# SewoongLab/PLeaS-Merging

Hardware: AMD Instinct MI355X
Metric: wall-clock (s): ResNet-101 pair, 100-batch act-match + 400-step PLeaS, 1/8 GPU (lower is better)
Workload: dtype f32

## Files before the change

include/pleas_hip.h:

```cpp
#ifndef PLEAS_HIP_H
#define PLEAS_HIP_H

#include <stddef.h>
#include <stdint.h>

#ifdef __cplusplus
extern "C" {
#endif

#define PLEAS_OK 0
#define PLEAS_EINVAL (-22)
#define PLEAS_ENOMEM (-12)
#define PLEAS_EHIP (-5)

const char* pleas_version(void);
const char* pleas_last_error(void);

#define PLEAS_EPI_INNER 0
#define PLEAS_EPI_NEG_CDIST 1
size_t pleas_gram_ws_bytes(int B, int C, int64_t HW);
int pleas_gram_accum(const float* x, const float* y, int B, int C, int64_t HW, int epilogue, int accumulate,
                     float* acc, void* ws, size_t ws_bytes, void* stream);

typedef struct pleas_gram_node {
// ... 10 lines not shown
    const float* scale_y;
    const float* shift_y;
} pleas_gram_node;
size_t pleas_gram_batch_ws_bytes(const pleas_gram_node* nodes, int n_nodes, const int* group_C, int n_groups);
int pleas_gram_batch(const pleas_gram_node* nodes, int n_nodes, float* const* group_acc, const int* group_C,
                     int n_groups, int epilogue, int accumulate, void* ws, size_t ws_bytes, int ws_fresh, void* stream);

#define PLEAS_LSAP_MAX_N 4096
int pleas_lsap_batched(const float* const* cost, const int* n, int nprob, int maximize, int64_t* const* col_ind,
                       void* stream);
int pleas_lsap_host(const void* cost, int is_double, int n, int maximize, int64_t* col_ind);

size_t pleas_bottleneck_ws_bytes(const int* n, int nprob);
int pleas_bottleneck_batched(const float* const* cost, const int* n, int nprob, int maximize, int64_t* const* col_ind,
                             float* t_out, void* ws, size_t ws_bytes, void* stream);
int pleas_bottleneck_host(const void* cost, int is_double, int n, int maximize, int64_t* col_ind, double* t_out);

int pleas_merge_blocks(const float* w1, const float* w2, float* out, int64_t outer, int rows_out, int cols_out,
                       int64_t inner, int rows_src, int cols_src, const int32_t* row1, const int32_t* row2,
                       const int32_t* col1, const int32_t* col2, int n_merged_rows, void* stream);

typedef struct pleas_merge_item {
    const float* w1;
    const float* w2;
    float* out;
    const int32_t* row1;
    const int32_t* row2;
    int64_t outer, inner;
    int rows_out, rows_src, n_merged;
    int sub_stride, sub_h, sub_w;
} pleas_merge_item;
size_t pleas_merge_batch_ws_bytes(const pleas_merge_item* items, int n_items);
int pleas_merge_batch(const pleas_merge_item* items, int n_items, void* ws, size_t ws_bytes, int ws_fresh, void* stream);

int pleas_bn_act(const float* x, const float* scale, const float* shift, const float* res, float* y, int64_t n,
                 int channels, int64_t inner, int relu, void* stream);
int pleas_bn_act_tracked(const float* x, const float* scale, const float* shift, const float* res, float* y_bn,
                         float* y_sum, float* y, int64_t n, int channels, int64_t inner, int relu, void* stream);

int pleas_bn_act_tracked_batches(const float* x, const float* scale, const float* shift, const float* res, float* y_bn,
                                 float* y_sum, float* y, int64_t n_per_batch, int batches, int channels, int64_t inner,
                                 int relu, void* stream);

int pleas_bn_act_maxpool(const float* x, const float* scale, const float* shift, float* y, int64_t n, int channels, int H,
                         int W, int KH, int KW, int stride, int pad, int relu, void* stream);

int pleas_pool_gather(const float* x, const int32_t* src, float* y, int64_t N, int C, int64_t HW, int K, void* stream);

int pleas_top1_count(const float* logits, const int64_t* labels, int64_t N, int C, int64_t* hits, int64_t* pred, void* stream);

int pleas_softmax_xent(const float* logits, const int64_t* labels, int64_t N, int C, float scale, float* dlogits,
                       float* row_loss, float* loss, int64_t* counts, void* stream);

size_t pleas_bn_train_ws_bytes(int64_t n, int channels);
int pleas_bn_train_fold(const float* x, int64_t n, int channels, int64_t inner, const float* gamma, const float* beta,
                        double eps, double momentum, float* running_mean, float* running_var,
                        int64_t* num_batches_tracked, float* scale, float* shift, void* ws, size_t ws_bytes,
                        void* stream);
int pleas_bn_train_fold_batches(const float* x, int64_t n, int batches, int channels, int64_t inner, const float* gamma,
                                const float* beta, double eps, double momentum, float* running_mean, float* running_var,
                                int64_t* num_batches_tracked, float* scale, float* shift, void* ws, size_t ws_bytes,
                                void* stream);

int pleas_masked_adam(float* p, const float* g, const float* mask, float* m, float* v, int64_t n, float lr,
                      float b1, float b2, float eps, int step, void* stream);

// ... 112 lines not shown
```

pleas_merging_amd/_lib.py:

```python
from __future__ import annotations

import ctypes
import os
from ctypes import POINTER, c_char_p, c_float, c_int, c_int64, c_size_t, c_void_p
from typing import Optional

_LIB: Optional[ctypes.CDLL] = None
LIB_PATH = os.path.join(os.path.dirname(os.path.abspath(__file__)), "csrc", "libpleas_hip.so")

EPI_INNER, EPI_NEG_CDIST = 0, 1
ARITH_FP32, ARITH_SPLIT_BF16, ARITH_SPLIT_BF16_EXACT = 0, 1, 2
LSAP_MAX_N = 4096
IMAGE_NHWC, IMAGE_NCHW = 0, 1

SIGNATURES = {
    "pleas_version": (c_char_p, []),
    "pleas_last_error": (c_char_p, []),
    "pleas_gram_ws_bytes": (c_size_t, [c_int, c_int, c_int64]),
    "pleas_gram_accum": (c_int, [c_void_p, c_void_p, c_int, c_int, c_int64, c_int, c_int, c_void_p, c_void_p, c_size_t,
                                 c_void_p]),
    "pleas_lsap_batched": (c_int, [POINTER(c_void_p), POINTER(c_int), c_int, c_int, POINTER(c_void_p), c_void_p]),
    "pleas_lsap_host": (c_int, [c_void_p, c_int, c_int, c_int, c_void_p]),
    "pleas_bottleneck_ws_bytes": (c_size_t, [POINTER(c_int), c_int]),
    "pleas_bottleneck_batched": (c_int, [POINTER(c_void_p), POINTER(c_int), c_int, c_int, POINTER(c_void_p), c_void_p, c_void_p,
                                         c_size_t, c_void_p]),
    "pleas_bottleneck_host": (c_int, [c_void_p, c_int, c_int, c_int, c_void_p, c_void_p]),
    "pleas_merge_blocks": (c_int, [c_void_p, c_void_p, c_void_p, c_int64, c_int, c_int, c_int64, c_int, c_int, c_void_p,
                                   c_void_p, c_void_p, c_void_p, c_int, c_void_p]),
    "pleas_merge_batch_ws_bytes": (c_size_t, [c_void_p, c_int]),
    "pleas_merge_batch": (c_int, [c_void_p, c_int, c_void_p, c_size_t, c_int, c_void_p]),
    "pleas_bn_act": (c_int, [c_void_p, c_void_p, c_void_p, c_void_p, c_void_p, c_int64, c_int, c_int64, c_int, c_void_p]),
    "pleas_bn_act_tracked": (c_int, [c_void_p, c_void_p, c_void_p, c_void_p, c_void_p, c_void_p, c_void_p, c_int64, c_int,
                                     c_int64, c_int, c_void_p]),
    "pleas_bn_act_maxpool": (c_int, [c_void_p, c_void_p, c_void_p, c_void_p, c_int64, c_int, c_int, c_int, c_int, c_int, c_int,
                                     c_int, c_int, c_void_p]),
    "pleas_bn_act_tracked_batches": (c_int, [c_void_p, c_void_p, c_void_p, c_void_p, c_void_p, c_void_p, c_void_p, c_int64, c_int,
                                             c_int, c_int64, c_int, c_void_p]),
    "pleas_bn_train_fold_batches": (c_int, [c_void_p, c_int64, c_int, c_int, c_int64, c_void_p, c_void_p, ctypes.c_double,
                                            ctypes.c_double, c_void_p, c_void_p, c_void_p, c_void_p, c_void_p, c_void_p,
                                            c_size_t, c_void_p]),
    "pleas_bn_train_ws_bytes": (c_size_t, [c_int64, c_int]),
    "pleas_bn_train_fold": (c_int, [c_void_p, c_int64, c_int, c_int64, c_void_p, c_void_p, ctypes.c_double, ctypes.c_double,
                                    c_void_p, c_void_p, c_void_p, c_void_p, c_void_p, c_void_p, c_size_t, c_void_p]),
    "pleas_masked_adam": (c_int, [c_void_p, c_void_p, c_void_p, c_void_p, c_void_p, c_int64, c_float, c_float, c_float,
                                  c_float, c_int, c_void_p]),
    "pleas_sqerr_ws_bytes": (c_size_t, [c_int64]),
    "pleas_sqerr": (c_int, [c_void_p, c_void_p, c_int64, c_float, c_int, c_void_p, c_float, c_void_p, c_void_p, c_size_t,
                            c_void_p]),
    "pleas_channel_sum": (c_int, [c_void_p, c_int, c_int, c_int64, c_void_p, c_void_p]),
    "pleas_linear_ws_bytes": (c_size_t, [c_int64, c_int, c_int]),
    "pleas_linear_plan_info": (c_int, [c_int64, c_int, c_int, POINTER(c_int)]),
    "pleas_linear_fwd": (c_int, [c_void_p, c_void_p, c_void_p, c_void_p, c_int64, c_int, c_int, c_void_p, c_size_t, c_void_p]),
    "pleas_column_sum": (c_int, [c_void_p, c_int64, c_int, c_void_p, c_void_p]),
    "pleas_image_batch": (c_int, [c_void_p, c_void_p, c_void_p, c_void_p, c_void_p, c_int64] + [c_int] * 6 + [c_void_p]),
    "pleas_resample_plan_bytes": (c_size_t, [c_void_p, c_int64, c_int, c_int]),
    "pleas_resample_plan": (c_int, [c_void_p, c_void_p, c_int64, c_int, c_int, c_int, c_int64, c_void_p, c_size_t]),
    "pleas_resample_plan_info": (c_int, [c_void_p, c_size_t, POINTER(c_int64)]),
    "pleas_image_resample_host": (c_int, [c_void_p, c_void_p, c_size_t, c_void_p, c_void_p, c_void_p, c_void_p]),
    "pleas_image_resample": (c_int, [c_void_p, c_void_p, c_void_p, c_size_t, c_void_p, c_void_p, c_void_p, c_void_p, c_size_t,
                                     c_void_p]),
    "pleas_prof_enable": (None, [c_int]),
    "pleas_prof_select": (None, [ctypes.c_uint]),
    "pleas_prof_reset": (None, []),
# ... 95 lines not shown
```

pleas_merging_amd/csrc/common.hpp:

```cpp
#pragma once
#include <hip/hip_runtime.h>

#include <cstdint>
#include <cstdio>
#include <algorithm>
#include <cstdlib>
#include <cstring>
#include <vector>

#include "pleas_hip.h"

namespace pleas {

extern thread_local char g_last_error[256];

inline int hip_fail(hipError_t e, const char* what) {
    std::snprintf(g_last_error, sizeof(g_last_error), "%s: %s", what, hipGetErrorString(e));
    return PLEAS_EHIP;
}

inline int bad_arg(const char* what) {
    std::snprintf(g_last_error, sizeof(g_last_error), "invalid argument: %s", what);
    return PLEAS_EINVAL;
}
// ... 144 lines not shown
            if (t.bytes) PLEAS_HIP_CHECK(hipMemcpyAsync((char*)ws + t.offset, t.host, t.bytes, hipMemcpyHostToDevice, stream));
        PLEAS_HIP_CHECK(hipStreamSynchronize(stream));
        p.uploaded = true;
        return PLEAS_OK;
    }
};

template <int N>
struct SideStreams {
    struct Set {
        hipStream_t streams[N];
        hipEvent_t forked, joined[N];
        bool ok = false;
    };
    static constexpr int kMaxDev = 16;
    Set sets[kMaxDev], none;
    bool tried[kMaxDev] = {false};
    Set& current() {
        int dev = 0;
        if (hipGetDevice(&dev) != hipSuccess || dev < 0 || dev >= kMaxDev) return none;
        Set& s = sets[dev];
        if (!tried[dev]) {
            tried[dev] = true;
            bool ok = hipEventCreateWithFlags(&s.forked, hipEventDisableTiming) == hipSuccess;
            for (int i = 0; ok && i < N; ++i)
                ok = hipStreamCreateWithFlags(&s.streams[i], hipStreamNonBlocking) == hipSuccess &&
                     hipEventCreateWithFlags(&s.joined[i], hipEventDisableTiming) == hipSuccess;
            s.ok = ok;
        }
        return s;
    }
};

template <class Item>
struct XcdWork {
    double w;
    int64_t key;
    Item it;
};
template <class Item>
inline std::vector<Item> xcd_order_items(std::vector<XcdWork<Item>>& work, const Item& noop, bool by_default = true) {
    std::vector<Item> out;
    const char* env = std::getenv("PLEAS_XCD_ORDER");
    if (env ? env[0] == '0' : !by_default) {
        std::stable_sort(work.begin(), work.end(), [](const XcdWork<Item>& a, const XcdWork<Item>& b) { return a.w > b.w; });
        for (auto& x : work) out.push_back(x.it);
        return out;
    }
    struct Group { double total = 0, longest = 0; std::vector<size_t> idx; };
    std::vector<Group> groups;
    {
        std::vector<size_t> order(work.size());
        for (size_t i = 0; i < work.size(); ++i) order[i] = i;
        std::stable_sort(order.begin(), order.end(), [&](size_t a, size_t b) { return work[a].key < work[b].key; });
        int64_t last = 0;
        for (size_t n = 0; n < order.size(); ++n) {
            const size_t i = order[n];
            if (n == 0 || work[i].key != last) groups.emplace_back();
            last = work[i].key;
            Group& g = groups.back();
            g.total += work[i].w;
            g.longest = std::max(g.longest, work[i].w);
            g.idx.push_back(i);
        }
    }
    std::stable_sort(groups.begin(), groups.end(), [](const Group& a, const Group& b) { return a.total > b.total; });
// ... 27 lines not shown
```

pleas_merging_amd/csrc/conv_fwd.hip:

```cpp
#include <algorithm>
#include <mutex>
#include <vector>

#include "fwd_schedule.hpp"
#include "nt_tile.hpp"

namespace pleas {

typedef short s16x4_t __attribute__((ext_vector_type(4)));
typedef short s16x8_t __attribute__((ext_vector_type(8)));

constexpr int fTN = 128;

enum class FwdMode : int { Fit = 0, Conv = 1, ConvImage = 2, Image = 3, ConvStats = 4 };
constexpr int fModes = 5;
constexpr bool fwd_has_target(FwdMode m) { return m == FwdMode::Fit; }
constexpr bool fwd_has_image(FwdMode m) { return m == FwdMode::ConvImage || m == FwdMode::Image; }
constexpr bool fwd_stores_y(FwdMode m) { return m != FwdMode::Image; }
constexpr bool fwd_has_stats(FwdMode m) { return m == FwdMode::ConvStats; }

struct FwdLayerDev {
    const float* ip;
    const float* w;
    const float* bias;
// ... 893 lines not shown
    d.KH = l.KH; d.KW = l.KW; d.stride = l.stride; d.pad = l.pad; d.Csrc = l.Csrc; d.n_merged = l.n_merged;
    d.HWo = (uint32_t)HWo; d.Ptot = (uint32_t)Ptot; d.Kd = (uint32_t)Kd;
    d.dscale = l.dscale;
    const int TM = l.Cout > 64 ? 128 : 64;
    d.variant = (TM == 64 ? 1 : 0) | (Kd % 4 == 0 ? 0 : 2);
    if (l.flags & PLEAS_FWD_KPOS_MAJOR) {
        if (l.Cin % kBK != 0) return bad_arg("conv_fwd: kernel-position-major weights need Cin % 32 == 0");
        d.variant |= 4;
    }
    lds_bytes = (size_t)(2 * TM * kLds + 2 * fTN * kLds) * sizeof(float);
    {
        const int R = l.KH * l.KW;
        const bool same = l.stride == 1 && l.KH == l.KW && (l.KH & 1) && l.pad == (l.KH - 1) / 2;
        const int halo = l.pad * (l.Win + 1);
        const int kind = R > 1 ? 2 : (HWo % 4 == 0 ? 0 : 1);
        const int Lr = kind == 2 ? fFlatColsK : fFlatRow1;
        const size_t flat_lds = std::max((size_t)(2 * TM * kLds + (kind == 2 ? fFlatColsK * fFlatPix : 2 * kBK * Lr)) * sizeof(float),
                                         (size_t)TM * 132 * sizeof(float));
        if (same && l.Cin % kBK == 0 && R <= 32 && (R == 1 || (l.flags & PLEAS_FWD_KPOS_MAJOR)) &&
            fTN + 2 * halo < Lr && flat_lds <= lds_bytes && (int64_t)l.N * l.Cin * HWo < (1ll << 32)) {
            d.variant |= 8 | (kind << 4);
            lds_bytes = flat_lds;
            if (arith_mode() != 0 && kind != 1) {
                const size_t img = (size_t)(TM * kSplitRow + (kind == 2 ? fFlatColsK * kSplitRow : 3 * kBK * fSplitPixRow)) * sizeof(__bf16);
                lds_bytes = std::max(img, (size_t)TM * 132 * sizeof(float));
            }
        }
    }
    TM_out = TM;
    return PLEAS_OK;
}

static std::mutex g_fplan_mu;

static int build_fwd_plan(FwdPlan& P, const pleas_fwd_layer* ly, int n) {
    P.split = arith_mode();
    P.layers.assign(n, FwdLayerDev());
    P.items.clear();
    for (int f = 0; f < fForms; ++f) P.form_begin[f] = P.form_count[f] = 0;
    P.loss.assign(n, FwdLossDev());
    P.flops = P.bytes = 0;
    std::vector<XcdWork<FwdItemDev>> work[fForms];
    double form_work[fForms] = {0};
    for (int f = 0; f < fForms; ++f) P.form_lds[f] = 0;
    int parts = 0;
    for (int i = 0; i < n; ++i) {
        const pleas_fwd_layer& l = ly[i];
        FwdLayerDev& d = P.layers[i];
        size_t lds_bytes = 0;
        int TM = 128;
        if (const int rc = fwd_describe(l, d, lds_bytes, TM); rc != PLEAS_OK) return rc;
        const int64_t Ptot = d.Ptot, Kd = d.Kd;
        d.part_base = parts;
        const int tms = (int)ceil_div(l.Cout, TM), tps = (int)ceil_div(Ptot, fTN);
        int slot = 0;
        const int form = fwd_form_of(d.variant);
        for (int tp = 0; tp < tps; ++tp)
            for (int tm = 0; tm < tms; ++tm) {
                XcdWork<FwdItemDev> w;
                w.it = FwdItemDev{i, tm, tp, slot++};
                w.w = (double)ceil_div(Kd, kBK) * TM;
                w.key = (int64_t)i * 65536 + tp / 32;
                work[form].push_back(w);
                form_work[form] += w.w;
            }
        P.loss[i] = FwdLossDev{parts, slot, l.loss_scale, 0};
// ... 301 lines not shown
```

pleas_merging_amd/csrc/merge_batch.hip:

```cpp
#include <algorithm>
#include <mutex>
#include <vector>

#include "common.hpp"

namespace pleas {

typedef float f32x4 __attribute__((ext_vector_type(4)));

constexpr int mThreads = 256;
constexpr int mUnroll = 4;
constexpr int mSpan = mThreads * mUnroll;

struct MergeItemDev {
    const float* w1;
    const float* w2;
    float* out;
    const int32_t* row1;
    const int32_t* row2;
    uint32_t total_v;
    uint32_t inner_v;
    uint32_t rows_out, rows_src;
    int n_merged, vec;
    int first_block;
    int stride;
    uint32_t w_out, w_src, inner_src, pad;
};

__global__ __launch_bounds__(mThreads) void merge_batch_kernel(const MergeItemDev* __restrict__ items,
                                                               const int* __restrict__ block_item) {
    const MergeItemDev it = items[block_item[blockIdx.x]];
    const uint32_t base = (uint32_t)(blockIdx.x - it.first_block) * mSpan + threadIdx.x;
    uint32_t idx[mUnroll];
    int r1[mUnroll], r2[mUnroll];
    uint32_t o_[mUnroll], iv_[mUnroll], r_[mUnroll];
#pragma unroll
    for (int u = 0; u < mUnroll; ++u) {
        idx[u] = base + u * mThreads;
        const uint32_t id = min(idx[u], it.total_v - 1);
        const uint32_t t = id / it.inner_v;
        iv_[u] = id - t * it.inner_v;
        o_[u] = t / it.rows_out;
        r_[u] = t - o_[u] * it.rows_out;
        r1[u] = PLEAS_GLOBAL_I(it.row1)[r_[u]];
        r2[u] = PLEAS_GLOBAL_I(it.row2)[r_[u]];
    }
    if (it.vec == 4) {
        f32x4 a[mUnroll], b[mUnroll];
#pragma unroll
        for (int u = 0; u < mUnroll; ++u) {
            const size_t oa = ((size_t)o_[u] * it.rows_src + max(r1[u], 0)) * it.inner_v + iv_[u];
            const size_t ob = ((size_t)o_[u] * it.rows_src + max(r2[u], 0)) * it.inner_v + iv_[u];
            a[u] = reinterpret_cast<const __attribute__((address_space(1))) f32x4*>(PLEAS_GLOBAL(it.w1))[oa];
            b[u] = reinterpret_cast<const __attribute__((address_space(1))) f32x4*>(PLEAS_GLOBAL(it.w2))[ob];
        }
#pragma unroll
        for (int u = 0; u < mUnroll; ++u) {
            if (idx[u] >= it.total_v) continue;
            const float coef = (int)r_[u] < it.n_merged ? 0.5f : 1.0f;
            f32x4 q;
#pragma unroll
            for (int e = 0; e < 4; ++e) q[e] = ((r1[u] >= 0 ? a[u][e] : 0.f) + (r2[u] >= 0 ? b[u][e] : 0.f)) * coef;
            reinterpret_cast<__attribute__((address_space(1))) f32x4*>(PLEAS_GLOBAL_W(it.out))[idx[u]] = q;
        }
    } else {
        float a[mUnroll], b[mUnroll];
#pragma unroll
        for (int u = 0; u < mUnroll; ++u) {
            uint32_t src = iv_[u], row_len = it.inner_v;
            if (it.stride > 0) {
                const uint32_t oh = iv_[u] / it.w_out, ow = iv_[u] - oh * it.w_out;
                src = (oh * it.w_src + ow) * (uint32_t)it.stride;
                row_len = it.inner_src;
            }
            a[u] = PLEAS_GLOBAL(it.w1)[((size_t)o_[u] * it.rows_src + max(r1[u], 0)) * row_len + src];
            b[u] = PLEAS_GLOBAL(it.w2)[((size_t)o_[u] * it.rows_src + max(r2[u], 0)) * row_len + src];
        }
#pragma unroll
        for (int u = 0; u < mUnroll; ++u) {
            if (idx[u] >= it.total_v) continue;
            const float coef = (int)r_[u] < it.n_merged ? 0.5f : 1.0f;
            PLEAS_GLOBAL_W(it.out)[idx[u]] = ((r1[u] >= 0 ? a[u] : 0.f) + (r2[u] >= 0 ? b[u] : 0.f)) * coef;
        }
    }
}

constexpr int mPtrBatch = 90;
struct MergePtrBatch {
    int base, count;
    const float* w1[mPtrBatch];
    const float* w2[mPtrBatch];
    float* out[mPtrBatch];
    const int32_t* row1[mPtrBatch];
    const int32_t* row2[mPtrBatch];
};
__global__ void merge_set_ptrs_kernel(MergeItemDev* __restrict__ items, const MergePtrBatch b) {
    const int t = blockIdx.x * blockDim.x + threadIdx.x;
    if (t < b.count) {
        MergeItemDev& d = items[b.base + t];
        d.w1 = b.w1[t];
        d.w2 = b.w2[t];
        d.out = b.out[t];
        d.row1 = b.row1[t];
        d.row2 = b.row2[t];
    }
}

struct MergePlan {
    std::vector<int64_t> key;
    std::vector<MergeItemDev> items;
    std::vector<int> block_item;
    size_t off_items = 0, off_blocks = 0, total = 0;
    double bytes = 0;
    bool uploaded = false;
};
static PlanCache<MergePlan, 1> g_mplans;
static std::mutex g_mplan_mu;
// ... 22 lines not shown
        d.total_v = (uint32_t)total_v;
        d.inner_v = (uint32_t)inner_v;
        d.rows_out = (uint32_t)m.rows_out;
        d.rows_src = (uint32_t)m.rows_src;
        d.n_merged = m.n_merged;
        d.vec = vec ? 4 : 1;
        d.stride = sub ? m.sub_stride : 0;
        d.w_out = (uint32_t)sub_wo;
        d.w_src = sub ? (uint32_t)m.sub_w : 0u;
        d.inner_src = sub ? (uint32_t)(m.sub_h * m.sub_w) : 0u;
        d.first_block = (int)P.block_item.size();
        const int64_t nb = ceil_div(total_v, mSpan);
        for (int64_t b = 0; b < nb; ++b) P.block_item.push_back(i);
        P.bytes += 3.0 * (double)(m.outer * m.rows_out * m.inner) * sizeof(float);
    }
    P.off_items = 0;
    P.off_blocks = align256(P.items.size() * sizeof(MergeItemDev));
    P.total = P.off_blocks + align256(P.block_item.size() * sizeof(int));
    P.uploaded = false;
    return PLEAS_OK;
}

}

using namespace pleas;

extern "C" size_t pleas_merge_batch_ws_bytes(const pleas_merge_item* items, int n_items) {
    if (!items || n_items <= 0) return 0;
    MergePlan tmp;
    if (build_merge_plan(tmp, items, n_items) != PLEAS_OK) return 0;
    return std::max<size_t>(tmp.total, 256);
}

extern "C" int pleas_merge_batch(const pleas_merge_item* items, int n_items, void* ws, size_t ws_bytes, int ws_fresh,
                                 void* stream_) {
    if (!items || n_items <= 0) return bad_arg("merge_batch: empty tensor list");
    for (int i = 0; i < n_items; ++i) {
        const pleas_merge_item& m = items[i];
        if (!m.w1 || !m.w2 || !m.out || !m.row1 || !m.row2) return bad_arg("merge_batch: null pointer");
        if (m.sub_stride <= 1 && m.inner % 4 == 0 && ((((uintptr_t)m.w1 | (uintptr_t)m.w2 | (uintptr_t)m.out) & 15) != 0))
            return bad_arg("merge_batch: tensors with inner % 4 == 0 must be 16-byte aligned");
    }
    hipStream_t stream = (hipStream_t)stream_;
    std::lock_guard<std::mutex> lk(g_mplan_mu);
    std::vector<int64_t> key;
    key.push_back(n_items);
    key.push_back((int64_t)(uintptr_t)ws);
    for (int i = 0; i < n_items; ++i) {
        const pleas_merge_item& m = items[i];
        for (int64_t v : {m.outer, m.inner, (int64_t)m.rows_out, (int64_t)m.rows_src, (int64_t)m.n_merged, (int64_t)m.sub_stride,
                          (int64_t)m.sub_h, (int64_t)m.sub_w})
            key.push_back(v);
    }
    MergePlan* hit = nullptr;
    if (const int rc = g_mplans.get(key, hit, [&](MergePlan& p) { return build_merge_plan(p, items, n_items); }); rc != PLEAS_OK)
        return rc;
    MergePlan& P = *hit;
    if (P.block_item.empty()) return PLEAS_OK;
    if (const int rc = g_mplans.prepare(P, "merge_batch", ws, ws_bytes, ws_fresh, stream, [&] {
            return std::vector<PlanTable>{plan_table(P.off_items, P.items), plan_table(P.off_blocks, P.block_item)};
        });
        rc != PLEAS_OK)
        return rc;
    char* base = (char*)ws;
    MergeItemDev* di = reinterpret_cast<MergeItemDev*>(base + P.off_items);
    for (int b0 = 0; b0 < n_items; b0 += mPtrBatch) {
        MergePtrBatch pb;
        pb.base = b0;
        pb.count = std::min(mPtrBatch, n_items - b0);
        for (int t = 0; t < pb.count; ++t) {
            const pleas_merge_item& m = items[b0 + t];
            pb.w1[t] = m.w1; pb.w2[t] = m.w2; pb.out[t] = m.out; pb.row1[t] = m.row1; pb.row2[t] = m.row2;
        }
        hipLaunchKernelGGL(merge_set_ptrs_kernel, dim3(1), dim3(128), 0, stream, di, pb);
        PLEAS_LAUNCH_CHECK("merge_set_ptrs_kernel");
    }
    {
        ProfScope prof(kProfMergeBlocks, 0.0, P.bytes, stream);
        hipLaunchKernelGGL(merge_batch_kernel, dim3((unsigned)P.block_item.size()), dim3(mThreads), 0, stream, di,
                           reinterpret_cast<const int*>(base + P.off_blocks));
    }
    PLEAS_LAUNCH_CHECK("merge_batch_kernel");
    return PLEAS_OK;
}
```

pleas_merging_amd/hip_ops.py:

```python
from __future__ import annotations

import contextlib
import ctypes
import math
import os
import threading
from typing import List, Optional, Sequence, Tuple

import numpy as np
import torch

from . import _lib
from ._lib import ARITH_FP32, ARITH_SPLIT_BF16, ARITH_SPLIT_BF16_EXACT, EPI_INNER, EPI_NEG_CDIST, PleasHipError, check


class _Pinned(threading.local):

    depth = 0
    handle = 0


_PINNED = _Pinned()


# ... 590 lines not shown
    check(rc, "pleas_loss_final")


class MergeBatch(_GroupedLaunch):

    STRUCT, WS_BYTES, LAUNCH = _lib.MergeItem, "pleas_merge_batch_ws_bytes", "pleas_merge_batch"

    def add(self, w1: torch.Tensor, w2: torch.Tensor, row_axis: int, row1: torch.Tensor, row2: torch.Tensor,
            n_merged_rows: int, out: Optional[torch.Tensor] = None, subsample: int = 1) -> torch.Tensor:
        if w1.shape != w2.shape or not w1.is_cuda or w1.dtype != torch.float32 or w2.dtype != torch.float32:
            raise PleasHipError("MergeBatch.add: fp32 CUDA sources of equal shape expected")
        w1, w2 = w1.contiguous(), w2.contiguous()
        shape = list(w1.shape)
        row_axis = row_axis % w1.dim()
        rows_out = int(row1.numel())
        want = shape[:row_axis] + [rows_out] + shape[row_axis + 1:]
        sub = (0, 0, 0)
        if subsample > 1:
            if w1.dim() != 4 or row_axis != 1:
                raise PleasHipError("MergeBatch.add: subsample needs [N, C, H, W] sources merged along axis 1")
            sub = (int(subsample), shape[2], shape[3])
            want = want[:2] + [-(-shape[2] // subsample), -(-shape[3] // subsample)]
        if out is None:
            out = torch.empty(want, dtype=torch.float32, device=w1.device)
        elif list(out.shape) != want or out.dtype != torch.float32 or not out.is_contiguous() or out.device != w1.device:
            raise PleasHipError("MergeBatch.add: out must be a contiguous fp32 tensor of shape %s" % (want,))
        self._queue((w1, w2, out, row1, row2), (math.prod(shape[:row_axis]), math.prod(want[row_axis + 1:]), rows_out,
                                                shape[row_axis], int(n_merged_rows)) + sub)
        return out

    def _fill(self, a, tensors, geo) -> None:
        a.w1, a.w2, a.out, a.row1, a.row2 = (t.data_ptr() for t in tensors)
        a.outer, a.inner, a.rows_out, a.rows_src, a.n_merged, a.sub_stride, a.sub_h, a.sub_w = geo


def fwd_plan_lanes() -> dict:
    ms, lane, items = (ctypes.c_double * 10)(), (ctypes.c_int * 10)(), (ctypes.c_int * 10)()
    state = _lib.lib().pleas_fwd_plan_lanes(ms, lane, items)
    return {"state": state, "forms": {f: {"ms": round(ms[f], 4), "lane": lane[f], "items": items[f]} for f in range(10) if items[f]}}


class FwdBatch(_GroupedLaunch):

    STRUCT, WS_BYTES, LAUNCH = _lib.FwdLayer, "pleas_fwd_batch_ws_bytes", "pleas_fwd_batch"
    KPOS_MAJOR = 1

    def add(self, ip, w, bias, o1, o2, row1, row2, n_merged: int, resid, dscale: float, loss_scale: float,
            kernel=(1, 1), stride: int = 1, pad: int = 0, flags: int = 0) -> None:
        for t in (ip, w, o1, o2, resid):
            if not t.is_contiguous():
                raise PleasHipError("FwdBatch.add: contiguous tensors expected")
        N, Cin = ip.shape[0], ip.shape[1]
        Hin, Win = (ip.shape[2], ip.shape[3]) if ip.dim() == 4 else (1, 1)
        self._queue((ip, w, bias, o1, o2, row1, row2, resid),
                    (N, w.shape[0], Cin, Hin, Win, kernel[0], kernel[1], stride, pad, o1.shape[1], int(n_merged),
                     float(dscale), float(loss_scale), int(flags)))

    def _fill(self, a, tensors, geo) -> None:
        a.ip, a.w, a.bias, a.o1, a.o2, a.row1, a.row2, a.resid = (t.data_ptr() if t is not None else None for t in tensors)
        (a.N, a.Cout, a.Cin, a.Hin, a.Win, a.KH, a.KW, a.stride, a.pad, a.Csrc, a.n_merged, a.dscale, a.loss_scale,
         a.flags) = geo

    def _launch_args(self, loss: torch.Tensor) -> tuple:
        if loss.numel() != len(self._arr) or not loss.is_contiguous():
            raise PleasHipError("FwdBatch: loss must hold one float per layer")
        return (loss.data_ptr(),)
# ... 615 lines not shown
```

pleas_merging_amd/methods/pleas_merging.py:

```python
from __future__ import annotations

import contextlib
import math
from typing import Dict, List, Optional, Tuple

import torch
import torch.nn.functional as F
from torch import nn

from .. import hip_ops
from ..core.utils import Axis, get_attr
from .data_parallel import _SPIN, _emulated_collective, _force_collectives, dp_all_gather_, dp_reduce_scatter_, dp_slice, dp_sum_
from .frozen_sources import (ActivationTap, FrozenSources, Generation, SourceTaps, TapDict, _TapView,
                             prepare_sources, tap_pointers)
from .partial_matching import block_maps, get_blocks, spread_blocks


def get_gradient_mask(perm_blocks, model_weights: Dict[str, nn.Module]) -> List[torch.Tensor]:
    masks = []
    for name, layer in model_weights.items():
        frozen = _frozen_blocks(perm_blocks, name)
        for p in layer.parameters():
            mask = torch.ones_like(p)
            if p.dim() >= 2:
                for rows, cols in frozen:
                    mask[rows, cols] = 0.0
            masks.append(mask)
    return masks


def _frozen_blocks(perm_blocks, name: str):
    bi = perm_blocks.get(Axis("%s.weight" % name, 1))
    bo = perm_blocks.get(Axis("%s.weight" % name, 0))
    ni, mi = (len(bi[0]), len(bi[2])) if bi is not None else (3, 0)
    no, mo = (len(bo[0]), len(bo[2])) if bo is not None else (1000, 0)
    return ((slice(ni, ni + mi), slice(no + mo, no + 2 * mo)), (slice(ni + mi, ni + 2 * mi), slice(no, no + mo)))


def _square_conv(mod: nn.Conv2d) -> bool:
    return (mod.groups == 1 and mod.dilation == (1, 1) and mod.stride[0] == mod.stride[1]
            and mod.padding[0] == mod.padding[1] and mod.kernel_size[0] == mod.kernel_size[1])


def cosine_lrs(base_lr: float, t_max: int, n: int) -> List[float]:
    lrs, lr = [], base_lr
    for t in range(n):
        if t > 0:
            if (t - 1 - t_max) % (2 * t_max) == 0:
# ... 182 lines not shown
                            run.append(cand)
                        else:
                            break
                    if group > 1 and (len(run) == group or (exhausted and len(run) > 1 and len(run) == len(ahead))):
                        sources.launch_group(run)
                        del ahead[:len(run)]
                    else:
                        sources.enqueue(ahead.pop(0))
                    sources.stage(ahead[:group])
                if not queue:
                    break
                self.step(queue[0].batch)
            yield idx
            idx += 1

    @torch.no_grad()
    def step(self, x: torch.Tensor, next_x: Optional[torch.Tensor] = None) -> None:
        with self._session():
            self._step(x, next_x)

    def finish(self) -> nn.Module:
        sd = self.model3.state_dict()
        for plan in self.plans:
            sd["%s.weight" % plan.name] = (plan.w.detach().permute(0, 3, 1, 2) if plan.kpos else plan.w.detach()).clone()
            if plan.b is not None:
                sd["%s.bias" % plan.name] = plan.b.detach().clone()
        self.model3.load_state_dict(sd)
        self.sources.close()
        return self.model3


class _UpdateRecord:

    __slots__ = ("key", "bufs", "names", "fwd_rows", "fwd_loss", "fwd_index", "bias_grads", "vendor_losses", "merge_tab", "fwd_tab", "complete")

    def __init__(self, key: tuple, bufs: dict):
        self.key, self.bufs = key, bufs
        self.fwd_rows, self.bias_grads, self.vendor_losses = [], [], []
        self.names = self.fwd_loss = self.fwd_index = self.merge_tab = self.fwd_tab = None
        self.complete = bool(key)


class PleasFitter(_LayerFitter):

    def __init__(self, model1, model2, model3, spec, perm, costs, budget_ratios, max_steps: int, lr: float = 5e-4, *args, **kwargs):
        super().__init__(model1, model2, model3, spec, perm, costs, budget_ratios, max_steps, lr, *args, **kwargs)
        like = lambda arena, t: None if arena is None or t is None else \
            arena[t.storage_offset():t.storage_offset() + t.numel()].view(t.shape)
        for plan in self.plans:
            plan.gw, plan.gb, plan.gw2, plan.gb2 = like(self.g, plan.w), like(self.g, plan.b), like(self.g2, plan.w), like(self.g2, plan.b)
        self.lrs = cosine_lrs(lr, max_steps, max_steps + 1)
        self.step_count = 0
        self.loss_now = self._g_ext[self.p.numel():]
        self.loss_sum = torch.zeros(len(self.plans), dtype=torch.float32, device=self.device)
        self.fwd = self.ops.FwdBatch(self.device)
        self._buffers: Dict[tuple, Dict[tuple, Tuple[torch.Tensor, torch.Tensor]]] = {}
        self._loss_bufs: Dict[tuple, Tuple[torch.Tensor, torch.Tensor]] = {}
        self._replay: Optional[_UpdateRecord] = None
        self.fast_updates = 0

    def _lay_out_arenas(self, total: int, shard_optimizer: Optional[bool]) -> None:
        self.shard_optimizer = (shard_optimizer is None or bool(shard_optimizer)) and (self.world > 1 or _force_collectives())
        if self.shard_optimizer:
            total = (total + 4 * self.world - 1) // (4 * self.world) * (4 * self.world)
        self._shard = total // self.world if self.shard_optimizer else total
        super()._lay_out_arenas(total, shard_optimizer)
        dev = self.device
        self._g_ext = torch.zeros(total + len(self.layer_modules), dtype=torch.float32, device=dev)
        self.g = self._g_ext[:total]
        self.g2 = torch.zeros(total, dtype=torch.float32, device=dev) if self.stacked else None
        self.m = torch.zeros(self._shard, dtype=torch.float32, device=dev)
        self.v = torch.zeros(self._shard, dtype=torch.float32, device=dev)
        self._g_shard = torch.zeros(self._shard, dtype=torch.float32, device=dev) if self.shard_optimizer else None

    def _fit_layer(self, idx: int, plan: _LayerPlan, rec: _UpdateRecord) -> None:
        ops, name, mod, cout = self.ops, plan.name, plan.mod, plan.w_shape[0]
        ip1, ip2 = (t[name] for t in self.gen.taps.inputs)
        o1, o2 = (t[name] for t in self.gen.taps.outputs)
        if not (_square_conv(mod) if plan.is_conv else ip1.dim() == 2):
            self._fit_layer_vendor(idx, plan, rec)
            return
        geo = (tuple(mod.kernel_size), mod.stride[0], mod.padding[0]) if plan.is_conv else ((1, 1), 1, 0)
        sub = geo[1] if (plan.is_conv and geo[0] == (1, 1) and geo[1] > 1 and geo[2] == 0) else 1
        if sub > 1:
            geo = ((1, 1), 1, 0)
        for h, (in_maps, (r1, r2, nm)) in enumerate(plan.halves):
            if cout != r1.numel():
                raise RuntimeError("layer %s: %d merged outputs vs %d target blocks" % (name, cout, r1.numel()))
            if in_maps[0].numel() != plan.w_shape[1]:
                raise RuntimeError("layer %s: %d merged inputs vs %d input blocks" % (name, plan.w_shape[1], in_maps[0].numel()))
            kept = rec.bufs.get((idx, h))
            ip = self.merge.add(ip1, ip2, 1, *in_maps, out=kept[0] if kept else None, subsample=sub)
            resid = kept[1] if kept else torch.empty((ip.shape[0], cout) + tuple(o1.shape[2:]), dtype=torch.float32,
                                                     device=ip.device)
            if kept is None:
                rec.bufs[(idx, h)] = (ip, resid)
            n = resid.numel() * len(plan.halves) * self.world
            self.fwd.add(ip, plan.w, plan.b, o1, o2, r1, r2, nm, resid, 2.0 / n, 1.0 / n, *geo,
                         flags=ops.FwdBatch.KPOS_MAJOR if plan.kpos else 0)
            rec.fwd_rows.append(idx)
            gw, gb = (plan.gw, plan.gb) if h == 0 else (plan.gw2, plan.gb2)
            self.wgrad.add(resid, ip, gw, *geo, flags=ops.WgradBatch.KPOS_MAJOR if plan.kpos else 0)
            if gb is not None:
                rec.bias_grads.append((resid, plan, gb))

    def _fit_layer_vendor(self, idx: int, plan: _LayerPlan, rec: _UpdateRecord) -> None:
        ops, name, mod = self.ops, plan.name, plan.mod
        ip1, ip2 = (t[name] for t in self.gen.taps.inputs)
        o1, o2 = (t[name] for t in self.gen.taps.outputs)
        for h, (in_maps, out_maps) in enumerate(plan.halves):
            axis = 1 if plan.is_conv else ip1.dim() - 1
            ip = ops.merge_blocks(ip1, ip2, axis, *in_maps)
            op = ops.merge_blocks(o1, o2, axis, *out_maps)
            with torch.enable_grad():
                w = plan.w.detach().requires_grad_(True)
                b = plan.b.detach().requires_grad_(True) if plan.b is not None else None
                if plan.is_conv:
                    out = F.conv2d(ip, w, b, mod.stride, mod.padding, mod.dilation, mod.groups)
                else:
                    out = F.linear(ip, w, b)
                n = out.numel() * len(plan.halves) * self.world
                loss = ((out - op) ** 2).sum() / n
                grads = torch.autograd.grad(loss, [w] + ([b] if b is not None else []))
            gw, gb = (plan.gw, plan.gb) if h == 0 else (plan.gw2, plan.gb2)
            gw.copy_(grads[0])
            if b is not None:
                gb.copy_(grads[1])
            rec.vendor_losses.append((idx, loss.detach()))
        rec.complete = False

    def _bias_gradients(self, rec: _UpdateRecord) -> None:
        for resid, plan, gb in rec.bias_grads:
            self.ops.channel_sum(resid if resid.dim() > 1 else resid.reshape(1, -1), gb)

    def _update_key(self) -> tuple:
        first, taps = self.plans[0].name, self.gen.taps.taps1[0]
        if first not in taps:
            return ()
        n = (taps.hi - taps.lo) if isinstance(taps, _TapView) else taps[first].shape[0]
        return (n,) + tuple(self.gen.taps.x.shape[1:])

    def _step(self, x: torch.Tensor, next_x: Optional[torch.Tensor]) -> None:
        self._begin_update(x, next_x)
        key = self._update_key()
        rec = self._replay if (self._replay is not None and key and self._replay.key == key) else None
        ptrs = None
        if rec is not None:
            ptrs = [tap_pointers(t, rec.names) for t in self.gen.taps.inputs + self.gen.taps.outputs]
            if any(p is None for p in ptrs):
                rec = None
        if rec is not None:
            self._replay_update(rec, ptrs)
        else:
            self._replay = None
            rec = self._record_update(key)
            if rec.complete:
                self._replay = rec
        self._exchange_and_apply()
        self._end_update()

    def _record_update(self, key: tuple) -> _UpdateRecord:
        rec = _UpdateRecord(key, self._buffers.setdefault(key, {}) if key else {})
        in1, in2 = self.gen.taps.inputs
        with self.ops.pin_stream():
            for idx, plan in enumerate(self.plans):
                if plan.name not in in1 or plan.name not in in2:
                    print("Key error on %s" % plan.name)
                    rec.complete = False
                    continue
                self._fit_layer(idx, plan, rec)
        self.merge.flush()
        if rec.fwd_rows:
            rows = tuple(rec.fwd_rows)
            if rows not in self._loss_bufs:
                self._loss_bufs[rows] = (torch.zeros(len(rows), dtype=torch.float32, device=self.device),
                                         torch.tensor(rows, dtype=torch.long, device=self.device))
            rec.fwd_loss, rec.fwd_index = self._loss_bufs[rows]
            self.fwd.flush(rec.fwd_loss)
        self._scatter_losses(rec)
        self._bias_gradients(rec)
        n_wgrad = self.wgrad.pending()
        self.wgrad.flush()
        rec.complete = rec.complete and n_wgrad > 0
        if rec.complete:
            rec.names = tuple(self.plans[i].name for i in rec.fwd_rows)
            rec.merge_tab, rec.fwd_tab = self.merge.table(), self.fwd.table()
            rec.complete = (rec.merge_tab is not None and rec.fwd_tab is not None
                            and len(rec.merge_tab) == len(rec.fwd_tab) == len(rec.names))
        return rec

    def _replay_update(self, rec: _UpdateRecord, ptrs: list) -> None:
        rec.merge_tab["w1"][:], rec.merge_tab["w2"][:], rec.fwd_tab["o1"][:], rec.fwd_tab["o2"][:] = ptrs
        with self.ops.pin_stream():
            self.merge.relaunch()
            self.fwd.relaunch(rec.fwd_loss)
        self.fast_updates += 1
        self._scatter_losses(rec)
        self._bias_gradients(rec)
        with self.ops.pin_stream():
            self.wgrad.relaunch()

    def _scatter_losses(self, rec: _UpdateRecord) -> None:
        if rec.fwd_rows:
            if self.stacked:
                self.loss_now.zero_()
                self.loss_now.index_add_(0, rec.fwd_index, rec.fwd_loss)
            else:
                self.loss_now.index_copy_(0, rec.fwd_index, rec.fwd_loss)
        if rec.vendor_losses:
            if not rec.fwd_rows:
                self.loss_now.zero_()
            seen = set()
            for idx, loss in rec.vendor_losses:
                if idx in seen:
                    self.loss_now[idx] += loss
                else:
                    self.loss_now[idx] = loss
                    seen.add(idx)

    def _exchange_and_apply(self) -> None:
        if self.stacked:
            self.g.add_(self.g2)
        lr = self.lrs[min(self.step_count, len(self.lrs) - 1)]
        self.step_count += 1
        if self.shard_optimizer:
            lo, hi = self.rank * self._shard, (self.rank + 1) * self._shard
            g_mine = dp_reduce_scatter_(self.g, self._g_shard, self.rank, self.world)
            dp_sum_(self.loss_now, self.world)
            self.loss_sum.add_(self.loss_now)
            self.ops.masked_adam(self.p[lo:hi], g_mine, self.mask[lo:hi], self.m, self.v, lr, self.step_count)
            dp_all_gather_(self.p, self.rank, self.world)
        else:
            dp_sum_(self._g_ext, self.world)
# ... 37 lines not shown
```

Baseline: 5.850.

## Overlap next step's weight merge with weight-gradient kernels on a side stream

Double-buffers the merged interpolated-weight arena so that, during replayed updates, the merge for the next queued generation runs on an idle forward side stream while the current step's weight-gradient kernels run. The merge uses a grid-stride kernel with a capped block count so it shares the GPU instead of flooding it. The next step then skips its own merge launch and reads the prefetched buffer, joined through an event. This adds a second arena of memory, pointer-table bookkeeping and cross-stream event sync, and relies on the next generation's taps being ready and keyed identically.

```diff
diff --git a/include/pleas_hip.h b/include/pleas_hip.h
--- a/include/pleas_hip.h
+++ b/include/pleas_hip.h
@@ -66,6 +66,10 @@
 } pleas_merge_item;
 size_t pleas_merge_batch_ws_bytes(const pleas_merge_item* items, int n_items);
 int pleas_merge_batch(const pleas_merge_item* items, int n_items, void* ws, size_t ws_bytes, int ws_fresh, void* stream);
+int pleas_merge_batch_narrow(const pleas_merge_item* items, int n_items, void* ws, size_t ws_bytes, int ws_fresh,
+                             int max_blocks, void* stream);
+int pleas_merge_batch_beside(const pleas_merge_item* items, int n_items, void* ws, size_t ws_bytes, int ws_fresh, void* stream);
+int pleas_merge_beside_join(void* stream);
 
 int pleas_bn_act(const float* x, const float* scale, const float* shift, const float* res, float* y, int64_t n,
                  int channels, int64_t inner, int relu, void* stream);
diff --git a/pleas_merging_amd/_lib.py b/pleas_merging_amd/_lib.py
--- a/pleas_merging_amd/_lib.py
+++ b/pleas_merging_amd/_lib.py
@@ -29,6 +29,9 @@
                                    c_void_p, c_void_p, c_void_p, c_int, c_void_p]),
     "pleas_merge_batch_ws_bytes": (c_size_t, [c_void_p, c_int]),
     "pleas_merge_batch": (c_int, [c_void_p, c_int, c_void_p, c_size_t, c_int, c_void_p]),
+    "pleas_merge_batch_narrow": (c_int, [c_void_p, c_int, c_void_p, c_size_t, c_int, c_int, c_void_p]),
+    "pleas_merge_batch_beside": (c_int, [c_void_p, c_int, c_void_p, c_size_t, c_int, c_void_p]),
+    "pleas_merge_beside_join": (c_int, [c_void_p]),
     "pleas_bn_act": (c_int, [c_void_p, c_void_p, c_void_p, c_void_p, c_void_p, c_int64, c_int, c_int64, c_int, c_void_p]),
     "pleas_bn_act_tracked": (c_int, [c_void_p, c_void_p, c_void_p, c_void_p, c_void_p, c_void_p, c_void_p, c_int64, c_int,
                                      c_int64, c_int, c_void_p]),
diff --git a/pleas_merging_amd/csrc/common.hpp b/pleas_merging_amd/csrc/common.hpp
--- a/pleas_merging_amd/csrc/common.hpp
+++ b/pleas_merging_amd/csrc/common.hpp
@@ -200,6 +200,8 @@
     }
 };
 
+hipStream_t fwd_idle_lane(int lane);
+
 template <class Item>
 struct XcdWork {
     double w;
diff --git a/pleas_merging_amd/csrc/conv_fwd.hip b/pleas_merging_amd/csrc/conv_fwd.hip
--- a/pleas_merging_amd/csrc/conv_fwd.hip
+++ b/pleas_merging_amd/csrc/conv_fwd.hip
@@ -949,6 +949,12 @@
 }
 
 static std::mutex g_fplan_mu;
+
+hipStream_t fwd_idle_lane(int lane) {
+    std::lock_guard<std::mutex> lk(g_fplan_mu);
+    SideStreams<fLanes>::Set& side = g_fwd_side.current();
+    return side.ok && lane >= 0 && lane < fLanes ? side.streams[lane] : nullptr;
+}
 
 static int build_fwd_plan(FwdPlan& P, const pleas_fwd_layer* ly, int n) {
     P.split = arith_mode();
diff --git a/pleas_merging_amd/csrc/merge_batch.hip b/pleas_merging_amd/csrc/merge_batch.hip
--- a/pleas_merging_amd/csrc/merge_batch.hip
+++ b/pleas_merging_amd/csrc/merge_batch.hip
@@ -27,10 +27,9 @@
     uint32_t w_out, w_src, inner_src, pad;
 };
 
-__global__ __launch_bounds__(mThreads) void merge_batch_kernel(const MergeItemDev* __restrict__ items,
-                                                               const int* __restrict__ block_item) {
-    const MergeItemDev it = items[block_item[blockIdx.x]];
-    const uint32_t base = (uint32_t)(blockIdx.x - it.first_block) * mSpan + threadIdx.x;
+__device__ __forceinline__ void merge_unit(const MergeItemDev* __restrict__ items, const int* __restrict__ block_item, uint32_t unit) {
+    const MergeItemDev it = items[block_item[unit]];
+    const uint32_t base = (unit - (uint32_t)it.first_block) * mSpan + threadIdx.x;
     uint32_t idx[mUnroll];
     int r1[mUnroll], r2[mUnroll];
     uint32_t o_[mUnroll], iv_[mUnroll], r_[mUnroll];
@@ -83,6 +82,16 @@
             PLEAS_GLOBAL_W(it.out)[idx[u]] = ((r1[u] >= 0 ? a[u] : 0.f) + (r2[u] >= 0 ? b[u] : 0.f)) * coef;
         }
     }
+}
+
+__global__ __launch_bounds__(mThreads) void merge_batch_kernel(const MergeItemDev* __restrict__ items,
+                                                               const int* __restrict__ block_item) {
+    merge_unit(items, block_item, blockIdx.x);
+}
+
+__global__ __launch_bounds__(mThreads) void merge_batch_narrow_kernel(const MergeItemDev* __restrict__ items,
+                                                                      const int* __restrict__ block_item, uint32_t n_units) {
+    for (uint32_t unit = blockIdx.x; unit < n_units; unit += gridDim.x) merge_unit(items, block_item, unit);
 }
 
 constexpr int mPtrBatch = 90;
@@ -171,16 +180,14 @@
     return std::max<size_t>(tmp.total, 256);
 }
 
-extern "C" int pleas_merge_batch(const pleas_merge_item* items, int n_items, void* ws, size_t ws_bytes, int ws_fresh,
-                                 void* stream_) {
-    if (!items || n_items <= 0) return bad_arg("merge_batch: empty tensor list");
+static int merge_launch(const pleas_merge_item* items, int n_items, void* ws, size_t ws_bytes, int ws_fresh, int max_blocks,
+                        hipStream_t stream) {
     for (int i = 0; i < n_items; ++i) {
         const pleas_merge_item& m = items[i];
         if (!m.w1 || !m.w2 || !m.out || !m.row1 || !m.row2) return bad_arg("merge_batch: null pointer");
         if (m.sub_stride <= 1 && m.inner % 4 == 0 && ((((uintptr_t)m.w1 | (uintptr_t)m.w2 | (uintptr_t)m.out) & 15) != 0))
             return bad_arg("merge_batch: tensors with inner % 4 == 0 must be 16-byte aligned");
     }
-    hipStream_t stream = (hipStream_t)stream_;
     std::lock_guard<std::mutex> lk(g_mplan_mu);
     std::vector<int64_t> key;
     key.push_back(n_items);
@@ -214,11 +221,83 @@
         hipLaunchKernelGGL(merge_set_ptrs_kernel, dim3(1), dim3(128), 0, stream, di, pb);
         PLEAS_LAUNCH_CHECK("merge_set_ptrs_kernel");
     }
+    const int* block_item = reinterpret_cast<const int*>(base + P.off_blocks);
+    const unsigned n_units = (unsigned)P.block_item.size();
     {
         ProfScope prof(kProfMergeBlocks, 0.0, P.bytes, stream);
-        hipLaunchKernelGGL(merge_batch_kernel, dim3((unsigned)P.block_item.size()), dim3(mThreads), 0, stream, di,
-                           reinterpret_cast<const int*>(base + P.off_blocks));
+        if (max_blocks > 0)
+            hipLaunchKernelGGL(merge_batch_narrow_kernel, dim3(std::min(n_units, (unsigned)max_blocks)), dim3(mThreads), 0, stream, di,
+                               block_item, n_units);
+        else
+            hipLaunchKernelGGL(merge_batch_kernel, dim3(n_units), dim3(mThreads), 0, stream, di, block_item);
     }
     PLEAS_LAUNCH_CHECK("merge_batch_kernel");
     return PLEAS_OK;
 }
+
+extern "C" int pleas_merge_batch(const pleas_merge_item* items, int n_items, void* ws, size_t ws_bytes, int ws_fresh,
+                                 void* stream_) {
+    if (!items || n_items <= 0) return bad_arg("merge_batch: empty tensor list");
+    return merge_launch(items, n_items, ws, ws_bytes, ws_fresh, 0, (hipStream_t)stream_);
+}
+
+extern "C" int pleas_merge_batch_narrow(const pleas_merge_item* items, int n_items, void* ws, size_t ws_bytes, int ws_fresh,
+                                        int max_blocks, void* stream_) {
+    if (n_items == 0) return PLEAS_OK;
+    if (!items || n_items < 0) return bad_arg("merge_batch_narrow: null tensor list");
+    if (max_blocks <= 0) return bad_arg("merge_batch_narrow: max_blocks must be positive");
+    return merge_launch(items, n_items, ws, ws_bytes, ws_fresh, max_blocks, (hipStream_t)stream_);
+}
+
+constexpr int kMergeBesideBlocks = 1024;
+constexpr int kMergeBesideLane = 0;
+namespace {
+struct BesideEvents {
+    hipEvent_t forked, done;
+    bool tried = false, ok = false, pending = false;
+};
+BesideEvents g_beside[16];
+std::mutex g_beside_mu;
+BesideEvents* beside_events() {
+    int dev = 0;
+    if (hipGetDevice(&dev) != hipSuccess || dev < 0 || dev >= 16) return nullptr;
+    BesideEvents& e = g_beside[dev];
+    if (!e.tried) {
+        e.tried = true;
+        e.ok = hipEventCreateWithFlags(&e.forked, hipEventDisableTiming) == hipSuccess &&
+               hipEventCreateWithFlags(&e.done, hipEventDisableTiming) == hipSuccess;
+    }
+    return e.ok ? &e : nullptr;
+}
+int beside_blocks() {
+    const char* env = std::getenv("PLEAS_MERGE_BESIDE_BLOCKS");
+    return std::max(1, env && env[0] ? std::atoi(env) : kMergeBesideBlocks);
+}
+}
+
+extern "C" int pleas_merge_batch_beside(const pleas_merge_item* items, int n_items, void* ws, size_t ws_bytes, int ws_fresh,
+                                        void* stream_) {
+    if (!items || n_items <= 0) return bad_arg("merge_batch_beside: empty tensor list");
+    hipStream_t stream = (hipStream_t)stream_;
+    static const int blocks = beside_blocks();
+    hipStream_t side = fwd_idle_lane(kMergeBesideLane);
+    std::lock_guard<std::mutex> lk(g_beside_mu);
+    BesideEvents* ev = beside_events();
+    if (!side || !ev || side == stream)
+        return merge_launch(items, n_items, ws, ws_bytes, ws_fresh, 0, stream);
+    PLEAS_HIP_CHECK(hipEventRecord(ev->forked, stream));
+    PLEAS_HIP_CHECK(hipStreamWaitEvent(side, ev->forked, 0));
+    const int rc = merge_launch(items, n_items, ws, ws_bytes, ws_fresh, blocks, side);
+    PLEAS_HIP_CHECK(hipEventRecord(ev->done, side));
+    ev->pending = true;
+    return rc;
+}
+
+extern "C" int pleas_merge_beside_join(void* stream_) {
+    std::lock_guard<std::mutex> lk(g_beside_mu);
+    BesideEvents* ev = beside_events();
+    if (!ev || !ev->pending) return PLEAS_OK;
+    PLEAS_HIP_CHECK(hipStreamWaitEvent((hipStream_t)stream_, ev->done, 0));
+    ev->pending = false;
+    return PLEAS_OK;
+}
diff --git a/pleas_merging_amd/hip_ops.py b/pleas_merging_amd/hip_ops.py
--- a/pleas_merging_amd/hip_ops.py
+++ b/pleas_merging_amd/hip_ops.py
@@ -646,6 +646,43 @@
     def _fill(self, a, tensors, geo) -> None:
         a.w1, a.w2, a.out, a.row1, a.row2 = (t.data_ptr() for t in tensors)
         a.outer, a.inner, a.rows_out, a.rows_src, a.n_merged, a.sub_stride, a.sub_h, a.sub_w = geo
+
+    def _launch_args(self, max_blocks: Optional[int] = None, beside: bool = False) -> tuple:
+        return ("beside",) if beside else (int(max_blocks),) if max_blocks is not None else ()
+
+    def _launch(self, fresh: int, extra: tuple) -> int:
+        lib, args = _lib.lib(), (self._arr, len(self._arr), self._ws.data_ptr(), self._ws.numel(), fresh)
+        if not extra:
+            return lib.pleas_merge_batch(*args, _stream())
+        if extra[0] == "beside":
+            return lib.pleas_merge_batch_beside(*args, _stream())
+        return lib.pleas_merge_batch_narrow(*args, extra[0], _stream())
+
+    def flush(self, max_blocks: Optional[int] = None) -> None:
+        self._flush(max_blocks)
+
+    def adopt(self, other: "MergeBatch") -> None:
+        if self._keep or other._arr is None:
+            raise PleasHipError("MergeBatch.adopt: nothing flushed yet, or entries pending")
+        n = len(other._arr)
+        self._arr = (self.STRUCT * n)()
+        ctypes.memmove(self._arr, other._arr, ctypes.sizeof(self._arr))
+        need = int(_lib.lib().pleas_merge_batch_ws_bytes(self._arr, n))
+        if need == 0:
+            raise PleasHipError("pleas_merge_batch_ws_bytes rejected the list: %s" % _lib.lib().pleas_last_error().decode())
+        self._ws = torch.empty(need, dtype=torch.uint8, device=self.device)
+        self._fresh = 1
+
+    def relaunch_beside(self) -> None:
+        if self._keep or self._arr is None or self._ws is None:
+            raise PleasHipError("MergeBatch.relaunch_beside: no table adopted or flushed, or entries pending")
+        rc = self._launch(self._fresh, ("beside",))
+        self._fresh = 0
+        check(rc, "pleas_merge_batch_beside")
+
+    @staticmethod
+    def join_beside() -> None:
+        check(_lib.lib().pleas_merge_beside_join(_stream()), "pleas_merge_beside_join")
 
 
 def fwd_plan_lanes() -> dict:
diff --git a/pleas_merging_amd/methods/pleas_merging.py b/pleas_merging_amd/methods/pleas_merging.py
--- a/pleas_merging_amd/methods/pleas_merging.py
+++ b/pleas_merging_amd/methods/pleas_merging.py
@@ -2,8 +2,10 @@
 
 import contextlib
 import math
+import os
 from typing import Dict, List, Optional, Tuple
 
+import numpy as np
 import torch
 import torch.nn.functional as F
 from torch import nn
@@ -14,6 +16,8 @@
 from .frozen_sources import (ActivationTap, FrozenSources, Generation, SourceTaps, TapDict, _TapView,
                              prepare_sources, tap_pointers)
 from .partial_matching import block_maps, get_blocks, spread_blocks
+
+_MERGE_BESIDE_DEFAULT = "1"
 
 
 def get_gradient_mask(perm_blocks, model_weights: Dict[str, nn.Module]) -> List[torch.Tensor]:
@@ -262,13 +266,15 @@
 
 class _UpdateRecord:
 
-    __slots__ = ("key", "bufs", "names", "fwd_rows", "fwd_loss", "fwd_index", "bias_grads", "vendor_losses", "merge_tab", "fwd_tab", "complete")
+    __slots__ = ("key", "bufs", "names", "fwd_rows", "fwd_loss", "fwd_index", "bias_grads", "vendor_losses", "merge_tab", "fwd_tab", "complete",
+                 "ips", "wgrad_tab", "ip_sets", "ip_ptrs", "turn")
 
     def __init__(self, key: tuple, bufs: dict):
         self.key, self.bufs = key, bufs
         self.fwd_rows, self.bias_grads, self.vendor_losses = [], [], []
         self.names = self.fwd_loss = self.fwd_index = self.merge_tab = self.fwd_tab = None
         self.complete = bool(key)
+        self.ips, self.wgrad_tab, self.ip_sets, self.ip_ptrs, self.turn = [], None, None, None, 0
 
 
 class PleasFitter(_LayerFitter):
@@ -288,6 +294,12 @@
         self._loss_bufs: Dict[tuple, Tuple[torch.Tensor, torch.Tensor]] = {}
         self._replay: Optional[_UpdateRecord] = None
         self.fast_updates = 0
+        self._ride = (os.environ.get("PLEAS_MERGE_BESIDE", _MERGE_BESIDE_DEFAULT) != "0" and self.world == 1
+                      and not self.shard_optimizer and self._upd_stream is not None)
+        self.merge_ahead = self.ops.MergeBatch(self.device)
+        self._ip_alt: Dict[tuple, torch.Tensor] = {}
+        self._ahead: Optional[Generation] = None
+        self.rides = 0
 
     def _lay_out_arenas(self, total: int, shard_optimizer: Optional[bool]) -> None:
         self.shard_optimizer = (shard_optimizer is None or bool(shard_optimizer)) and (self.world > 1 or _force_collectives())
@@ -325,6 +337,7 @@
                                                      device=ip.device)
             if kept is None:
                 rec.bufs[(idx, h)] = (ip, resid)
+            rec.ips.append(ip)
             n = resid.numel() * len(plan.halves) * self.world
             self.fwd.add(ip, plan.w, plan.b, o1, o2, r1, r2, nm, resid, 2.0 / n, 1.0 / n, *geo,
                          flags=ops.FwdBatch.KPOS_MAJOR if plan.kpos else 0)
@@ -363,12 +376,13 @@
         for resid, plan, gb in rec.bias_grads:
             self.ops.channel_sum(resid if resid.dim() > 1 else resid.reshape(1, -1), gb)
 
-    def _update_key(self) -> tuple:
-        first, taps = self.plans[0].name, self.gen.taps.taps1[0]
+    def _update_key(self, gen: Optional[Generation] = None) -> tuple:
+        gen = self.gen if gen is None else gen
+        first, taps = self.plans[0].name, gen.taps.taps1[0]
         if first not in taps:
             return ()
         n = (taps.hi - taps.lo) if isinstance(taps, _TapView) else taps[first].shape[0]
-        return (n,) + tuple(self.gen.taps.x.shape[1:])
+        return (n,) + tuple(gen.taps.x.shape[1:])
 
     def _step(self, x: torch.Tensor, next_x: Optional[torch.Tensor]) -> None:
         self._begin_update(x, next_x)
@@ -382,7 +396,7 @@
         if rec is not None:
             self._replay_update(rec, ptrs)
         else:
-            self._replay = None
+            self._replay = self._ahead = None
             rec = self._record_update(key)
             if rec.complete:
                 self._replay = rec
@@ -417,18 +431,62 @@
             rec.merge_tab, rec.fwd_tab = self.merge.table(), self.fwd.table()
             rec.complete = (rec.merge_tab is not None and rec.fwd_tab is not None
                             and len(rec.merge_tab) == len(rec.fwd_tab) == len(rec.names))
+        if rec.complete and self._ride:
+            self._second_set(rec)
         return rec
+
+    def _second_set(self, rec: _UpdateRecord) -> None:
+        rec.wgrad_tab = self.wgrad.table()
+        if rec.wgrad_tab is None or len(rec.wgrad_tab) != len(rec.ips) or len(rec.merge_tab) != len(rec.ips):
+            return
+        offs, total = [], 0
+        for ip in rec.ips:
+            offs.append(total)
+            total += (ip.numel() + 63) // 64 * 64
+        arena = self._ip_alt.get(rec.key)
+        if arena is None or arena.numel() != total:
+            arena = self._ip_alt[rec.key] = torch.empty(total, dtype=torch.float32, device=self.device)
+        rec.ip_sets = (list(rec.ips), [arena])
+        rec.ip_ptrs = (np.array([ip.data_ptr() for ip in rec.ips], dtype=np.uint64),
+                       np.uint64(arena.data_ptr()) + np.array(offs, dtype=np.uint64) * np.uint64(4))
+        self.merge_ahead.adopt(self.merge)
+        rec.turn = 1
 
     def _replay_update(self, rec: _UpdateRecord, ptrs: list) -> None:
         rec.merge_tab["w1"][:], rec.merge_tab["w2"][:], rec.fwd_tab["o1"][:], rec.fwd_tab["o2"][:] = ptrs
+        ahead, self._ahead = self._ahead, None
+        if rec.ip_ptrs is not None:
+            mine = rec.ip_ptrs[rec.turn]
+            rec.merge_tab["out"][:], rec.fwd_tab["ip"][:], rec.wgrad_tab["ip"][:] = mine, mine, mine
         with self.ops.pin_stream():
-            self.merge.relaunch()
+            if rec.ip_ptrs is not None and ahead is self.gen:
+                self.rides += 1
+            else:
+                self.merge.relaunch()
             self.fwd.relaunch(rec.fwd_loss)
         self.fast_updates += 1
         self._scatter_losses(rec)
         self._bias_gradients(rec)
         with self.ops.pin_stream():
+            riding = rec.ip_ptrs is not None and self._ride_next(rec)
             self.wgrad.relaunch()
+            if riding:
+                self.merge_ahead.join_beside()
+        if rec.ip_ptrs is not None:
+            rec.turn = 1 - rec.turn
+
+    def _ride_next(self, rec: _UpdateRecord) -> bool:
+        nxt = self.sources.queue[0] if self.sources.queue else None
+        if nxt is None or nxt.taps.events is not self.gen.taps.events or self._update_key(nxt) != rec.key:
+            return False
+        ptrs = [tap_pointers(t, rec.names) for t in nxt.taps.inputs]
+        if any(p is None for p in ptrs):
+            return False
+        tab = self.merge_ahead.table()
+        tab["w1"][:], tab["w2"][:], tab["out"][:] = ptrs[0], ptrs[1], rec.ip_ptrs[1 - rec.turn]
+        self.merge_ahead.relaunch_beside()
+        self._ahead = nxt
+        return True
 
     def _scatter_losses(self, rec: _UpdateRecord) -> None:
         if rec.fwd_rows:
```

Result: no change. 5.809 (median of 6 runs) (-0.7%).
